# multimodallearning/convexAdam

Measured on AMD Instinct MI355X. Metric: volume-pairs/sec (160x192x224 MIND convex+Adam(80it)), higher is better.
Workload: dtype f32

## Files before the change

convexadam_amd/csrc/cvx_common.h:

```cpp
#pragma once
#include <hip/hip_runtime.h>
#include <stdint.h>
#include <stdio.h>
#include <stdarg.h>

#include <mutex>

#include "convexadam_hip.h"

namespace cvx {

void set_error(const char* fmt, ...);
int fail(int code, const char* fmt, ...);
int check_last(const char* what);

#define CVX_REQUIRE(cond, ...)                                      \
    do {                                                            \
        if (!(cond)) return ::cvx::fail(CVX_ERR_INVALID_ARG, __VA_ARGS__); \
    } while (0)

static inline hipStream_t as_stream(void* s) { return reinterpret_cast<hipStream_t>(s); }
static inline size_t align_up(size_t v, size_t a) { return (v + a - 1) / a * a; }
static inline int cdiv(int a, int b) { return (a + b - 1) / b; }
static inline int64_t cdiv64(int64_t a, int64_t b) { return (a + b - 1) / b; }

template <typename KernelT>
static inline void ensure_dynamic_lds(KernelT kernel, size_t bytes, size_t& granted) {
    static std::mutex mu;
    std::lock_guard<std::mutex> lock(mu);
    if (bytes > granted) {
        (void)hipFuncSetAttribute(reinterpret_cast<const void*>(kernel), hipFuncAttributeMaxDynamicSharedMemorySize, (int)bytes);
        (void)hipGetLastError();
        granted = bytes;
    }
}

struct Carver {
    char* base = nullptr;
    size_t used = 0;
    Carver() = default;
    explicit Carver(void* p) : base(static_cast<char*>(p)) {}
    size_t take_bytes(size_t bytes) { const size_t off = align_up(used, 256); used = off + bytes; return off; }
    template <typename T> T* take(size_t count) { const size_t off = take_bytes(count * sizeof(T)); return base ? reinterpret_cast<T*>(base + off) : nullptr; }
};
static inline size_t ws_query(const Carver& m) { return m.used ? m.used + 256 : 0; }

#define CVX_OPTIONS(X) \
    X(mind_tiled,          "CVX_MIND_TILED",            0)   \
    X(mind_overlap,        "CVX_MIND_OVERLAP",          0)   \
    X(mm_tx,               "CVX_MM_TX",                 0)   \
    X(mm_slots,            "CVX_MM_SLOTS",            512)   \
    X(box_tiled,           "CVX_BOX_TILED",             0)   \
    X(no_prune,            "CVX_NO_PRUNE",              0)   \
    X(corr_unfused,        "CVX_CORR_UNFUSED",          0)   \
    X(corr_fused_all,      "CVX_CORR_FUSED_ALL",        0)   \
    X(prune_stream_above,  "CVX_PRUNE_STREAM_ABOVE",   -1)   \
    X(cf_census,           "CVX_CF_CENSUS",             0)   \
    X(cf_prio,             "CVX_CF_PRIO",             136)   \
    X(warp_flat,           "CVX_WARP_FLAT",             0)   \
    X(box_yt,              "CVX_BOX_YT",                8)   \
    X(box_wg_target,       "CVX_BOX_WG_TARGET",         0)   \
    X(box_xsplit,          "CVX_BOX_XSPLIT",           -1)   \
    X(box_cpt,             "CVX_BOX_CPT",               4)   \
    X(box_uneven,          "CVX_BOX_UNEVEN",          200)   \
    X(box_adam_role,       "CVX_BOX_ADAM_ROLE",         0)   \
    X(box_dpp,             "CVX_BOX_DPP",               0)   \
    X(box_pk,              "CVX_BOX_PK",                0)   \
    X(box_prio,            "CVX_BOX_PRIO",              0)   \
    X(label_pow_block,     "CVX_LABEL_POW_BLOCK",      32)   \
    X(census_ptr,          nullptr,                     0)   \
    X(mind_mean_threads,   "CVX_MIND_MEAN_THREADS",     0)   \
    X(edt_sequential,      "CVX_EDT_SEQUENTIAL",        0)   \
    X(warp_octant,         "CVX_WARP_OCTANT",           4)   \
    X(box_fwd_tile,        "CVX_BOX_FWD_TILE",         -1)   \
    X(box_bwd_tile,        "CVX_BOX_BWD_TILE",         -1)   \
    X(box_walk,            "CVX_BOX_WALK",              1)   \
    X(corr_dual,           "CVX_CORR_DUAL",             0)   \
    X(prune_refine,        "CVX_PRUNE_REFINE",          1)   \
    X(mind_records,        "CVX_MIND_RECORDS",          1)   \
    X(resize_up2,          "CVX_RESIZE_UP2",            1)   \
    X(mind_blocked,        "CVX_MIND_BLOCKED",          1)   \
    X(corr_cert,           "CVX_CORR_CERT",             1)   \
    X(cc_debug,            "CVX_CC_DEBUG",              0)   \
    X(ic_fused,            "CVX_IC_FUSED",              0)   \
    X(mind_single,         "CVX_MIND_SINGLE",           0)   \
    X(ms_zlen,             "CVX_MS_ZLEN",               0)   \
    X(cf_map,              "CVX_CF_MAP",                1)   \
    X(cert_unfused,        "CVX_CERT_UNFUSED",          0)   \
    X(fbox_tile,           "CVX_FBOX_TILE",             0)   \
    X(box_tile_sync,       "CVX_BOX_TILE_SYNC",         0)   \
    X(box_prediv,          "CVX_BOX_PREDIV",            1)   \
    X(tile_census_ptr,     nullptr,                     0)
#define X(name, env, dflt) long long name;
struct Options { CVX_OPTIONS(X) };
#undef X
Options& options();
const unsigned* adam_sqrt_table();
class ContextScope {
public:
    explicit ContextScope(const cvx_context* c);
    ~ContextScope();
    ContextScope(const ContextScope&) = delete;
    ContextScope& operator=(const ContextScope&) = delete;
private:
    void* prev_;
    bool active_;
};

#ifdef CVX_RACE_JITTER
__device__ __forceinline__ void cvx_jitter() {
    unsigned t = (unsigned)__builtin_amdgcn_s_memtime();
    t ^= (unsigned)__builtin_amdgcn_s_getreg((4 << 0) | (0 << 6) | (31 << 11)) * 2654435761u;
    t ^= t >> 13; t *= 0x9E3779B1u; t ^= t >> 15;
    const int n = (int)(t & 15);
    for (int i = 0; i < n; ++i) __builtin_amdgcn_s_sleep(1);
}
__device__ __forceinline__ void cvx_barrier() { cvx_jitter(); __syncthreads(); cvx_jitter(); }
#else
__device__ __forceinline__ void cvx_barrier() { __syncthreads(); }
#endif

__device__ __forceinline__ int clampi(int v, int lo, int hi) { return v < lo ? lo : (v > hi ? hi : v); }

__device__ __forceinline__ float fdiv(float a, float b) { return __fdiv_rn(a, b); }
__device__ __forceinline__ float fsqrt(float a) { return sqrtf(a); }

__device__ __forceinline__ float cvx_expf(float d) {
    const float R_LN2f = 1.442695040888963407359924681001892137426645954152985934135449406931f;
    const float L2Uf = 0.693145751953125f, L2Lf = 1.428606765330187045e-06f;
    const float qf = rintf(d * R_LN2f);
    const int q = (int)qf;
    float s = __builtin_fmaf(qf, -L2Uf, d);
    s = __builtin_fmaf(qf, -L2Lf, s);
    float u = 0.000198527617612853646278381f;
    u = __builtin_fmaf(u, s, 0.00139304355252534151077271f);
    u = __builtin_fmaf(u, s, 0.00833336077630519866943359f);
    u = __builtin_fmaf(u, s, 0.0416664853692054748535156f);
    u = __builtin_fmaf(u, s, 0.166666671633720397949219f);
    u = __builtin_fmaf(u, s, 0.5f);
    u = 1.0f + __builtin_fmaf(s * s, u, s);
    u = __builtin_ldexpf(u, q);
    if (d < -104.0f) u = 0.0f;
    if (d > 100.0f) u = __int_as_float(0x7f800000);
    return u;
}

struct ExpTable { const unsigned char* tbl; unsigned first, count; };
ExpTable mind_exp_table();

typedef float f32x4 __attribute__((ext_vector_type(4)));
typedef __attribute__((address_space(3))) f32x4 lds_f32x4;
__device__ __forceinline__ f32x4 lds_load4(const float* p) { return *(const volatile lds_f32x4*)p; }
__device__ __forceinline__ void lds_store4(float* p, f32x4 v) { *(volatile lds_f32x4*)p = v; }

typedef int i32x4 __attribute__((ext_vector_type(4)));
__device__ __forceinline__ float4 buffer_load16(__amdgpu_buffer_rsrc_t rsrc, unsigned lane_off, unsigned uni_off) {
    const i32x4 v = __builtin_bit_cast(i32x4, __builtin_amdgcn_raw_buffer_load_b128(rsrc, (int)lane_off, (int)uni_off, 0));
    return make_float4(__int_as_float(v.x), __int_as_float(v.y), __int_as_float(v.z), __int_as_float(v.w));
}

typedef float f32x2 __attribute__((ext_vector_type(2)));
typedef __attribute__((address_space(3))) f32x2 lds_f32x2;
__device__ __forceinline__ f32x2 lds_load2(const float* p) { return *(const volatile lds_f32x2*)p; }
__device__ __forceinline__ void lds_store2(float* p, f32x2 v) { *(volatile lds_f32x2*)p = v; }

template <int D>
__device__ __forceinline__ float div_exact(float x) {
    static_assert(D == 8 || D == 27 || D == 64 || D == 125 || D == 343, "divisor not verified");
    constexpr float r = 1.0f / (float)D;
    const float q = x * r;
    const float e = __builtin_fmaf(-(float)D, q, x);
    return __builtin_fmaf(e, r, q);
}
template <int D>
__device__ __forceinline__ float div_exact_inf(float x) { return __builtin_isinf(x) ? x : div_exact<D>(x); }

template <int N>
__device__ __forceinline__ float cascade_seq(const float (&v)[N]) {
    static_assert(N < 256, "two cascade levels");
    float a0 = 0.f, a1 = 0.f;
    int i = 0;
#pragma unroll
    for (; i + 16 <= N; i += 16) {
#pragma unroll
        for (int j = 0; j < 16; ++j) a0 += v[i + j];
        a1 += a0;
        a0 = 0.f;
    }
#pragma unroll
    for (; i < N; ++i) a0 += v[i];
    a0 += a1;
    return a0;
}
template <int N>
__device__ __forceinline__ float outer_sum_ilp(const float (&v)[N]) {
    static_assert(N / 4 < 16, "single cascade level inside the interleaved sums");
    float p[4] = {0.f, 0.f, 0.f, 0.f};
#pragma unroll
    for (int i = 0; i < N / 4; ++i)
#pragma unroll
        for (int k = 0; k < 4; ++k) p[k] += v[4 * i + k];
#pragma unroll
    for (int i = (N / 4) * 4; i < N; ++i) p[0] += v[i];
    p[0] += p[1];
    p[0] += p[2];
    p[0] += p[3];
    return p[0];
}

__device__ __forceinline__ unsigned long long pack_min_key(float v, unsigned idx) {
    unsigned b = __float_as_uint(v);
    b = (b & 0x80000000u) ? ~b : (b | 0x80000000u);
    if (v != v) b = 0u;
    return ((unsigned long long)b << 32) | idx;
}

struct Tri {
    float ix, iy, iz;
    int x0, y0, z0;
    float tnw, tne, tsw, tse, bnw, bne, bsw, bse;
};
__device__ __forceinline__ float unnormalize(float g, int S) { return ((g + 1.0f) * (float)S - 1.0f) * 0.5f; }
__device__ __forceinline__ void tri_setup(Tri& t, float gx, float gy, float gz, int h, int w, int d) {
    t.ix = unnormalize(gx, d);
    t.iy = unnormalize(gy, w);
    t.iz = unnormalize(gz, h);
    const float fx = floorf(t.ix), fy = floorf(t.iy), fz = floorf(t.iz);
    t.x0 = (int)fmaxf(fminf(fx, 1.0e9f), -1.0e9f);
    t.y0 = (int)fmaxf(fminf(fy, 1.0e9f), -1.0e9f);
    t.z0 = (int)fmaxf(fminf(fz, 1.0e9f), -1.0e9f);
    const float x1 = (float)(t.x0 + 1), y1 = (float)(t.y0 + 1), z1 = (float)(t.z0 + 1);
    const float x0f = (float)t.x0, y0f = (float)t.y0, z0f = (float)t.z0;
    t.tnw = (x1 - t.ix) * (y1 - t.iy) * (z1 - t.iz);
    t.tne = (t.ix - x0f) * (y1 - t.iy) * (z1 - t.iz);
    t.tsw = (x1 - t.ix) * (t.iy - y0f) * (z1 - t.iz);
    t.tse = (t.ix - x0f) * (t.iy - y0f) * (z1 - t.iz);
    t.bnw = (x1 - t.ix) * (y1 - t.iy) * (t.iz - z0f);
    t.bne = (t.ix - x0f) * (y1 - t.iy) * (t.iz - z0f);
    t.bsw = (x1 - t.ix) * (t.iy - y0f) * (t.iz - z0f);
    t.bse = (t.ix - x0f) * (t.iy - y0f) * (t.iz - z0f);
}
__device__ __forceinline__ bool inb3(int z, int y, int x, int h, int w, int d) {
    return z >= 0 && z < h && y >= 0 && y < w && x >= 0 && x < d;
}
__device__ __forceinline__ float tri_sample(const Tri& t, const float* __restrict__ vol, int h, int w, int d) {
    const int x0 = t.x0, y0 = t.y0, z0 = t.z0, x1 = x0 + 1, y1 = y0 + 1, z1 = z0 + 1;
    const bool zi0 = (unsigned)z0 < (unsigned)h, zi1 = (unsigned)z1 < (unsigned)h, yi0 = (unsigned)y0 < (unsigned)w,
               yi1 = (unsigned)y1 < (unsigned)w, xi0 = (unsigned)x0 < (unsigned)d, xi1 = (unsigned)x1 < (unsigned)d;
    const int zc0 = clampi(z0, 0, h - 1), zc1 = clampi(z1, 0, h - 1), yc0 = clampi(y0, 0, w - 1), yc1 = clampi(y1, 0, w - 1),
              xc0 = clampi(x0, 0, d - 1), xc1 = clampi(x1, 0, d - 1);
    const size_t r00 = ((size_t)zc0 * w + yc0) * d, r01 = ((size_t)zc0 * w + yc1) * d, r10 = ((size_t)zc1 * w + yc0) * d,
                 r11 = ((size_t)zc1 * w + yc1) * d;
    const float v0 = vol[r00 + xc0], v1 = vol[r00 + xc1], v2 = vol[r01 + xc0], v3 = vol[r01 + xc1], v4 = vol[r10 + xc0],
                v5 = vol[r10 + xc1], v6 = vol[r11 + xc0], v7 = vol[r11 + xc1];
    float o = 0.0f, n;
    n = o + v0 * t.tnw; o = (zi0 && yi0 && xi0) ? n : o;
    n = o + v1 * t.tne; o = (zi0 && yi0 && xi1) ? n : o;
    n = o + v2 * t.tsw; o = (zi0 && yi1 && xi0) ? n : o;
    n = o + v3 * t.tse; o = (zi0 && yi1 && xi1) ? n : o;
    n = o + v4 * t.bnw; o = (zi1 && yi0 && xi0) ? n : o;
    n = o + v5 * t.bne; o = (zi1 && yi0 && xi1) ? n : o;
    n = o + v6 * t.bsw; o = (zi1 && yi1 && xi0) ? n : o;
    n = o + v7 * t.bse; o = (zi1 && yi1 && xi1) ? n : o;
    return o;
}

__device__ __forceinline__ void lin_coef(int o, int in, int out, int& i0, int& i1, float& l0, float& l1) {
    if (in == out) { i0 = o; i1 = o; l0 = 1.0f; l1 = 0.0f; return; }
    const float ratio = fdiv((float)in, (float)out);
    float src = __builtin_fmaf(ratio, (float)o + 0.5f, -0.5f);
    src = src < 0.0f ? 0.0f : src;
    int a = (int)floorf(src);
    a = a > in - 1 ? in - 1 : a;
    float l = src - (float)a;
    l = l < 0.f ? 0.f : (l > 1.f ? 1.f : l);
    i0 = a;
    i1 = a + ((a < in - 1) ? 1 : 0);
    l1 = l;
    l0 = 1.0f - l;
}
__device__ __forceinline__ float resize_chain(const float (&v)[8], float pre_mul, float lx0, float lx1, float ly0, float ly1, float lz0,
                                              float lz1) {
    const float a0 = __builtin_fmaf(v[0] * pre_mul, lx0, (v[1] * pre_mul) * lx1);
    const float a1 = __builtin_fmaf(v[2] * pre_mul, lx0, (v[3] * pre_mul) * lx1);
    const float b0 = __builtin_fmaf(v[4] * pre_mul, lx0, (v[5] * pre_mul) * lx1);
    const float b1 = __builtin_fmaf(v[6] * pre_mul, lx0, (v[7] * pre_mul) * lx1);
    const float l0 = __builtin_fmaf(a0, ly0, a1 * ly1);
    const float l1 = __builtin_fmaf(b0, ly0, b1 * ly1);
    return __builtin_fmaf(l0, lz0, l1 * lz1);
}

struct FastDiv { unsigned d, m; };
static inline FastDiv fastdiv_make(int d) { FastDiv f; f.d = (unsigned)d; f.m = d <= 1 ? 0u : (unsigned)((((unsigned long long)1 << 32) + (unsigned)d - 1) / (unsigned)d); return f; }
__device__ __forceinline__ int fastdiv(int n, FastDiv f) { return f.d <= 1 ? n : (int)__umulhi((unsigned)n, f.m); }

void profile_mark_kernel(const char* name, hipStream_t s);

int launch_box_zero(const float* in, float* out, int C, int H, int W, int D, int k, bool backward, hipStream_t s);
int launch_smoother(const float* in, float* out, float* tmp, int C, int H, int W, int D, const cvx_smoother& sm, bool backward,
                    hipStream_t s);
int launch_argmin_keys(const void* ssd, bool f16, int K, size_t v, unsigned long long* keys, bool arm, hipStream_t s);
struct CoupledWs { unsigned long long* keys[3]; int* idx; float* smin; unsigned long long* list; int* counts; };
CoupledWs coupled_layout(Carver& cv, int h, int w, int d, int disp_hw);
int launch_argmin(const void* ssd, bool f16, const float* mesh, const float* u, float coef, bool coupled, int K, size_t v,
                  unsigned long long* keys, int64_t* argmin_out, hipStream_t s);
int launch_resize(const float* in, int C, int h, int w, int d, float* out, int H, int W, int D, float pre_mul,
                  float post_div, hipStream_t s);
int launch_resize2(const float* in, int C, int h, int w, int d, int H, int W, int D, float* scratch, float* out, int h2, int w2,
                   int d2, float post_div, hipStream_t s);
struct AdamConsts { float w1, b2, omb2, bc2s, neg_step; const unsigned* sqrt_tbl; };
__device__ __forceinline__ float adam_sqrt(float x, const unsigned* __restrict__ tbl) {
    float r = fsqrt(x);
    if (tbl) {
        const unsigned b = __float_as_uint(x), e = b >> 23, mant = b & 0x7fffffu;
        if (b != 0 && e < 255) {
            const unsigned key = e ? (((e & 1u) << 23) | mant) : ((1u << 24) | mant);
            const unsigned code = (tbl[key >> 4] >> ((key & 15u) * 2u)) & 3u;
            if (code) r = __uint_as_float(__float_as_uint(r) + (code == 1u ? 1u : 0xffffffffu));
        }
    }
    return r;
}
__device__ __forceinline__ bool argmin_better(float cost, float best) { return (cost < best) | ((cost != cost) & (best == best)); }
__device__ __forceinline__ void adam_update(float g, float& P, float& m, float& v, const AdamConsts& ac) {
    const float mm = __builtin_fmaf(ac.w1, g - m, m);
    float vv = v * ac.b2;
    vv = __builtin_fmaf(ac.omb2 * g, g, vv);
    const float den = fdiv(adam_sqrt(vv, ac.sqrt_tbl), ac.bc2s) + 1e-8f;
    P = P + fdiv(ac.neg_step * mm, den);
    m = mm;
    v = vv;
}
struct AdamRun {
    const float *F2, *M2; int C, h, w, d; float *P, *m, *v; float lambda_weight; int niter, step0; float cost_scale;
    const float *base_h, *base_w, *base_d; float *U, *grad_out; const int* snapshot_iters_host; int n_snap; float* snapshots;
    void* workspace; size_t workspace_bytes; void* stream;
    const cvx_smoother* sm = nullptr;
    bool keep_state = true;
    bool f16_features = false;
    int fast = 0;
    bool features_are_records = false;
};
int adam_run_impl(const AdamRun& r);
size_t adam_record_floats(int C, size_t V);
int coupled_convex_impl(const void* ssd, bool f16, const int64_t* argmin, const float* mesh, int h, int w, int d, int disp_hw, float* out,
                        bool argmin_is_exact, void* workspace, size_t workspace_bytes, void* stream,
                        const unsigned char* cmask = nullptr);
int coupled_convex_dual_impl(const void* ssdA, const int64_t* argminA, float* outA, void* wsA, const void* ssdB, bool f16, const int64_t* argminB,
                             float* outB, void* wsB, const float* mesh, int h, int w, int d, int disp_hw, size_t workspace_bytes,
                             void* stream, bool counts_zeroed = false);
bool mind_pooled_supported(int H, int W, int D, int g1, int g2);
int launch_mind_pooled(const float* img, int H, int W, int D, int radius, int dilation, int g1, float* out1, int g2, float* out2,
                       float* raw, void* workspace, size_t workspace_bytes, hipStream_t s, int records = 0);
bool mind_pooled_records_supported(int H, int W, int D, int g1, int g2);
size_t mind_pooled_raw_floats(int H, int W, int D, int g1, int g2);
int launch_label_pooled(const float* lab, int H, int W, int D, int C, const int* present, const float* weights, float mult, int g1, float* out1,
                        int g2, float* out2, hipStream_t s);
bool corr_box2_supported(int h, int w, int d, int px);
int launch_corr_box2(const float* raw, int K, int h, int w, int d, int px, float* ssd, hipStream_t s, bool fast = false);
bool corr_fused_supported(int C, int h, int w, int d, int hw);
void corr_fused_set_prep_hook(void (*hook)(hipStream_t));
int corr_fused_items(int C, int h, int w, int d, int hw);
bool corr_fused_tiled(int C, int h, int w, int d, int hw);
void corr_call_prep_hook(hipStream_t s);
size_t corr_fused_workspace_bytes(int C, int h, int w, int d, int hw);
int launch_corr_fused(const float* fix, const float* mov, int C, int h, int w, int d, int hw, int cost, int n_box, int fast, int f16,
                      void* ssd, void* workspace, size_t workspace_bytes, hipStream_t s);
int launch_corr_fused_dual(const float* fix, const float* mov, int C, int h, int w, int d, int hw, int cost, int n_box, int fast, int f16,
                           void* ssd, void* ssd_rev, void* workspace, size_t workspace_bytes, void* workspace_rev, hipStream_t s);
bool corr_cert_supported(int C, int h, int w, int d, int hw);
size_t corr_cert_workspace_bytes(int C, int h, int w, int d, int hw);
int launch_corr_cert(const float* fix, const float* mov, int C, int h, int w, int d, int hw, float* ssdu, void* workspace, size_t workspace_bytes,
                     hipStream_t s);
enum class CorrKernel { None, Fused, Round1, CertRole, CertStaged, CertRound1 };
struct CorrUse { bool variant, ic, no_prune; };
struct CorrPlan {
    CorrKernel exact;
    CorrKernel cert;
    bool cert_supported;
    bool fused_ws, staged_ws, cert_round1_ws;
    bool pair_cert;
    bool pair_dual, pair_dual_ws;
};
CorrPlan corr_plan(int C, int h, int w, int d, int hw, CorrUse use = CorrUse{false, false, false});
size_t corr_certfast_workspace_bytes(int C, int h, int w, int d, int hw);
int launch_corr_certfast(const float* fix, const float* mov, int C, int h, int w, int d, int hw, float* ssdu, void* workspace, size_t workspace_bytes,
                         hipStream_t s);
size_t corr_certify_workspace_bytes(int C, int h, int w, int d, int hw, bool plain = false);
int corr_certified_argmin(const float* ssdu, const float* fix, const float* mov, int C, int h, int w, int d, int hw, int64_t* argmin,
                          void* workspace, size_t workspace_bytes, hipStream_t s);
int coupled_convex_cert_impl(const float* ssduA, const float* fixA, const float* movA, float* outA, void* wsA, const float* ssduB, const float* fixB,
                             const float* movB, float* outB, void* wsB, const float* mesh, int C, int h, int w, int d, int hw, size_t workspace_bytes,
                             hipStream_t s, int stage = 0);
bool box3_march_supported(int d);
int launch_box3_march(const float* in, float* out, int h, int w, int d, bool backward, float* P, float* m, float* v,
                      AdamConsts ac, float* gsave, hipStream_t s);
bool box3_tile_fwd_supported(const float* in, const float* out, int h, int w, int d);
int launch_box3_tile_fwd(const float* in, float* out, int h, int w, int d, int variant, hipStream_t s);
int box3_tile_fwd_auto(int h, int w, int d);
bool box3_tile_supported(const float* in, const float* out, int h, int w, int d, const float* P, const float* m, const float* v, const float* gsave);
int launch_box3_tile(const float* in, float* out, int h, int w, int d, int variant, bool backward, float* P, float* m, float* v, AdamConsts ac,
                     float* gsave, bool prediv, hipStream_t s);
int launch_to_chunked(const float* in, int C, size_t V, float* out, bool half, hipStream_t s);
int launch_warp_grad(const float* Fcl, const float* Mcl, int C, int h, int w, int d, const float* U, const float* bh,
                     const float* bw, const float* bd, float gsc, float cH, float cW, float cD, float* gU, bool half, bool prediv, hipStream_t s);
int launch_warp_grad_fast(const float* Fcl, const float* Mcl, int C, int h, int w, int d, const float* U, const float* bh,
                          const float* bw, const float* bd, float gsc, float cH, float cW, float cD, float* gU, bool half, hipStream_t s);
int launch_box3_fast(const float* in, float* out, int h, int w, int d, float* P, float* m, float* v, double bc1, double bc2,
                     float* gsave, hipStream_t s);
bool boxchain_fast_supported(const cvx_smoother& sm, int h, int w, int d);
int launch_boxchain_fast(const float* in, float* out, int h, int w, int d, const cvx_smoother& sm, bool reverse, hipStream_t s);
int launch_adam_update_fast(const float* G, float* P, float* m, float* v, size_t n, double bc1, double bc2, hipStream_t s);

}
```

convexadam_amd/csrc/warp.hip:

```cpp
#include "cvx_common.h"

namespace cvx {

__global__ __launch_bounds__(256) void k_to_chunked(const float* __restrict__ in, int C, size_t V, float* __restrict__ out) {
    const size_t p = (size_t)blockIdx.x * blockDim.x + threadIdx.x;
    if (p > V) return;
    const int c0 = 4 * (int)blockIdx.y;
    float4 r = make_float4(0.f, 0.f, 0.f, 0.f);
    if (p < V) {
        const float* src = in + (size_t)c0 * V + p;
        r.x = src[0];
        if (c0 + 1 < C) r.y = src[V];
        if (c0 + 2 < C) r.z = src[2 * V];
        if (c0 + 3 < C) r.w = src[3 * V];
    }
    reinterpret_cast<float4*>(out)[(size_t)blockIdx.y * (V + 1) + p] = r;
}

typedef _Float16 h16x4 __attribute__((ext_vector_type(4)));
__global__ __launch_bounds__(256) void k_to_chunked_h(const float* __restrict__ in, int C, size_t V, uint2* __restrict__ out) {
    const size_t p = (size_t)blockIdx.x * blockDim.x + threadIdx.x;
    if (p > V) return;
    const int c0 = 4 * (int)blockIdx.y;
    float4 r = make_float4(0.f, 0.f, 0.f, 0.f);
    if (p < V) {
        const float* src = in + (size_t)c0 * V + p;
        r.x = src[0];
        if (c0 + 1 < C) r.y = src[V];
        if (c0 + 2 < C) r.z = src[2 * V];
        if (c0 + 3 < C) r.w = src[3 * V];
    }
    const h16x4 o = {(_Float16)r.x, (_Float16)r.y, (_Float16)r.z, (_Float16)r.w};
    out[(size_t)blockIdx.y * (V + 1) + p] = __builtin_bit_cast(uint2, o);
}
__device__ __forceinline__ float4 buffer_load8h(__amdgpu_buffer_rsrc_t rsrc, unsigned lane_off, unsigned uni_off) {
    const h16x4 v = __builtin_bit_cast(h16x4, __builtin_amdgcn_raw_buffer_load_b64(rsrc, (int)lane_off, (int)uni_off, 0));
    return make_float4((float)v.x, (float)v.y, (float)v.z, (float)v.w);
}

template <bool BUF, bool HALF = false, bool PREDIV = false>
__global__ __launch_bounds__(256) void k_warp_grad(const float* __restrict__ F2, const float* __restrict__ M2, int C, int CP,
                                                   int h, int w, int d, const float* __restrict__ U,
                                                   const float* __restrict__ bh, const float* __restrict__ bw,
                                                   const float* __restrict__ bd, float gsc, float cH, float cW, float cD,
                                                   float* __restrict__ gU, unsigned long long* __restrict__ census, FastDiv dx, FastDiv dy,
                                                   float sc0, float sc1, float sc2) {
    const size_t V = (size_t)h * w * d;
    if (census && threadIdx.x == 0) {
        census[4 * blockIdx.x] = __builtin_amdgcn_s_memrealtime();
        census[4 * blockIdx.x + 3] = __builtin_amdgcn_s_getreg((4 << 0) | (0 << 6) | (31 << 11)) | ((unsigned long long)__builtin_amdgcn_s_getreg((20 << 0) | (0 << 6) | (31 << 11)) << 32);
    }
    const int ntx = (d + 15) / 16, nty = (w + 3) / 4, ntz = (h + 3) / 4;
    const int per_xcd = (int)(gridDim.x >> 3);
    const int bid = __builtin_amdgcn_readfirstlane((int)blockIdx.x);
    const int tile = (bid & 7) * per_xcd + (bid >> 3);
    if (tile >= ntx * nty * ntz) return;
    const int trow = fastdiv(tile, dx), tbz = fastdiv(trow, dy);
    const int tbx = tile - trow * ntx, tby = trow - tbz * nty;
    const int x = tbx * 16 + (threadIdx.x & 15), y = tby * 4 + ((threadIdx.x >> 4) & 3), z = tbz * 4 + (threadIdx.x >> 6);
    if (x >= d || y >= w || z >= h) return;
    const unsigned p = (unsigned)((z * w + y) * d + x);
    const float uH = U[p], uW = U[V + p], uD = U[2 * V + p];
    Tri t;
    tri_setup(t, bd[x] + fdiv(uD, sc2), bw[y] + fdiv(uW, sc1), bh[z] + fdiv(uH, sc0), h, w, d);
    const int x0 = t.x0, y0 = t.y0, z0 = t.z0, x1 = x0 + 1, y1 = y0 + 1, z1 = z0 + 1;
    const float fx0 = (float)x0, fy0 = (float)y0, fz0 = (float)z0, fx1 = (float)x1, fy1 = (float)y1, fz1 = (float)z1;
    const bool zin0 = (unsigned)z0 < (unsigned)h, zin1 = (unsigned)z1 < (unsigned)h, yin0 = (unsigned)y0 < (unsigned)w,
               yin1 = (unsigned)y1 < (unsigned)w, xin0 = (unsigned)x0 < (unsigned)d, xin1 = (unsigned)x1 < (unsigned)d;
    const int r00 = (z0 * w + y0) * d, r01 = (z0 * w + y1) * d, r10 = (z1 * w + y0) * d, r11 = (z1 * w + y1) * d;
    constexpr unsigned REC = HALF ? 8u : 16u;
    const unsigned zero_rec = (unsigned)V * REC;
    unsigned off[8];
    off[0] = (zin0 && yin0 && xin0) ? (unsigned)(r00 + x0) * REC : zero_rec; off[1] = (zin0 && yin0 && xin1) ? (unsigned)(r00 + x1) * REC : zero_rec;
    off[2] = (zin0 && yin1 && xin0) ? (unsigned)(r01 + x0) * REC : zero_rec; off[3] = (zin0 && yin1 && xin1) ? (unsigned)(r01 + x1) * REC : zero_rec;
    off[4] = (zin1 && yin0 && xin0) ? (unsigned)(r10 + x0) * REC : zero_rec; off[5] = (zin1 && yin0 && xin1) ? (unsigned)(r10 + x1) * REC : zero_rec;
    off[6] = (zin1 && yin1 && xin0) ? (unsigned)(r11 + x0) * REC : zero_rec; off[7] = (zin1 && yin1 && xin1) ? (unsigned)(r11 + x1) * REC : zero_rec;
    const float wgt[8] = {t.tnw, t.tne, t.tsw, t.tse, t.bnw, t.bne, t.bsw, t.bse};
    const float ax[8] = {fy1 - t.iy, fy1 - t.iy, t.iy - fy0, t.iy - fy0, fy1 - t.iy, fy1 - t.iy, t.iy - fy0, t.iy - fy0};
    const float bx[8] = {fz1 - t.iz, fz1 - t.iz, fz1 - t.iz, fz1 - t.iz, t.iz - fz0, t.iz - fz0, t.iz - fz0, t.iz - fz0};
    const float ay[8] = {fx1 - t.ix, t.ix - fx0, fx1 - t.ix, t.ix - fx0, fx1 - t.ix, t.ix - fx0, fx1 - t.ix, t.ix - fx0};
    const float bz[8] = {fy1 - t.iy, fy1 - t.iy, t.iy - fy0, t.iy - fy0, fy1 - t.iy, fy1 - t.iy, t.iy - fy0, t.iy - fy0};
    float gix = 0.f, giy = 0.f, giz = 0.f;
    const unsigned foff = p * REC;
    const unsigned chunk_bytes = (unsigned)(V + 1) * REC;
    const __amdgpu_buffer_rsrc_t mr = __builtin_amdgcn_make_buffer_rsrc(const_cast<float*>(M2), 0, (int)(chunk_bytes * (unsigned)(CP / 4)), 0x00020000);
    const __amdgpu_buffer_rsrc_t fr = __builtin_amdgcn_make_buffer_rsrc(const_cast<float*>(F2), 0, (int)(chunk_bytes * (unsigned)(CP / 4)), 0x00020000);
    unsigned coff = 0;
    for (int c0 = 0; c0 < CP / 4; ++c0, coff += chunk_bytes) {
        float vv[8][4], fv[4];
#pragma unroll
        for (int k = 0; k < 8; ++k) {
            const float4 q = HALF ? buffer_load8h(mr, off[k], coff) : BUF ? buffer_load16(mr, off[k], coff) : *reinterpret_cast<const float4*>(reinterpret_cast<const char*>(M2) + (size_t)c0 * chunk_bytes + off[k]);
            vv[k][0] = q.x; vv[k][1] = q.y; vv[k][2] = q.z; vv[k][3] = q.w;
        }
        const float4 fq = HALF ? buffer_load8h(fr, foff, coff) : BUF ? buffer_load16(fr, foff, coff) : *reinterpret_cast<const float4*>(reinterpret_cast<const char*>(F2) + (size_t)c0 * chunk_bytes + foff);
        fv[0] = fq.x; fv[1] = fq.y; fv[2] = fq.z; fv[3] = fq.w;
#pragma unroll
        for (int j = 0; j < 4; ++j) {
            float wv = 0.0f;
#pragma unroll
            for (int k = 0; k < 8; ++k) wv += vv[k][j] * wgt[k];
            const float df = wv - fv[j];
            const float gOut = gsc * (2.0f * df);
            gix -= vv[0][j] * ax[0] * bx[0] * gOut; giy -= vv[0][j] * ay[0] * bx[0] * gOut; giz -= vv[0][j] * ay[0] * bz[0] * gOut;
            gix += vv[1][j] * ax[1] * bx[1] * gOut; giy -= vv[1][j] * ay[1] * bx[1] * gOut; giz -= vv[1][j] * ay[1] * bz[1] * gOut;
            gix -= vv[2][j] * ax[2] * bx[2] * gOut; giy += vv[2][j] * ay[2] * bx[2] * gOut; giz -= vv[2][j] * ay[2] * bz[2] * gOut;
            gix += vv[3][j] * ax[3] * bx[3] * gOut; giy += vv[3][j] * ay[3] * bx[3] * gOut; giz -= vv[3][j] * ay[3] * bz[3] * gOut;
            gix -= vv[4][j] * ax[4] * bx[4] * gOut; giy -= vv[4][j] * ay[4] * bx[4] * gOut; giz += vv[4][j] * ay[4] * bz[4] * gOut;
            gix += vv[5][j] * ax[5] * bx[5] * gOut; giy -= vv[5][j] * ay[5] * bx[5] * gOut; giz += vv[5][j] * ay[5] * bz[5] * gOut;
            gix -= vv[6][j] * ax[6] * bx[6] * gOut; giy += vv[6][j] * ay[6] * bx[6] * gOut; giz += vv[6][j] * ay[6] * bz[6] * gOut;
            gix += vv[7][j] * ax[7] * bx[7] * gOut; giy += vv[7][j] * ay[7] * bx[7] * gOut; giz += vv[7][j] * ay[7] * bz[7] * gOut;
        }
    }
    float g[3];
    g[0] = fdiv(((float)h / 2.0f) * giz, sc0);
    g[1] = fdiv(((float)w / 2.0f) * giy, sc1);
    g[2] = fdiv(((float)d / 2.0f) * gix, sc2);
    const unsigned sH = (unsigned)(w * d);
    const unsigned pxp = x < d - 1 ? p + 1 : p, pxm = x > 0 ? p - 1 : p, pzp = z < h - 1 ? p + sH : p, pzm = z > 0 ? p - sH : p,
                   pyp = y < w - 1 ? p + (unsigned)d : p, pym = y > 0 ? p - (unsigned)d : p;
    float nb[3][6];
    const __amdgpu_buffer_rsrc_t ur = __builtin_amdgcn_make_buffer_rsrc(const_cast<float*>(U), 0, (int)(12u * (unsigned)V), 0x00020000);
    const unsigned nboff[6] = {4u * pxp, 4u * pxm, 4u * pzp, 4u * pzm, 4u * pyp, 4u * pym};
#pragma unroll
    for (int a = 0; a < 3; ++a)
#pragma unroll
        for (int k = 0; k < 6; ++k) nb[a][k] = __builtin_bit_cast(float, __builtin_amdgcn_raw_buffer_load_b32(ur, (int)nboff[k], (int)(4u * (unsigned)V) * a, 0));
    const float uc3[3] = {uH, uW, uD};
#pragma unroll
    for (int a = 0; a < 3; ++a) {
        const float uc = uc3[a];
        float acc = g[a], t;
        t = acc + -(cD * (2.0f * (nb[a][0] - uc))); acc = x < d - 1 ? t : acc;
        t = acc +  (cD * (2.0f * (uc - nb[a][1]))); acc = x > 0 ? t : acc;
        t = acc + -(cH * (2.0f * (nb[a][2] - uc))); acc = z < h - 1 ? t : acc;
        t = acc +  (cH * (2.0f * (uc - nb[a][3]))); acc = z > 0 ? t : acc;
        t = acc + -(cW * (2.0f * (nb[a][4] - uc))); acc = y < w - 1 ? t : acc;
        t = acc +  (cW * (2.0f * (uc - nb[a][5]))); acc = y > 0 ? t : acc;
        (gU + (size_t)a * V)[p] = PREDIV ? (acc == 0.0f ? acc : div_exact<27>(acc)) : acc;
    }
    if (census && threadIdx.x == 0) census[4 * blockIdx.x + 2] = __builtin_amdgcn_s_memrealtime();
}


int launch_to_chunked(const float* in, int C, size_t V, float* out, bool half, hipStream_t s) {
    const int CP = (C + 3) / 4 * 4;
    if ((size_t)(CP / 4) * (V + 1) * 16 >= ((size_t)1 << 31)) return fail(CVX_ERR_UNSUPPORTED, "adam_run: control grid too large (%zu voxels x %d channels)", V, C);
    if (half) hipLaunchKernelGGL(k_to_chunked_h, dim3((unsigned)cdiv64((int64_t)(V + 1), 256), CP / 4), dim3(256), 0, s, in, C, V, reinterpret_cast<uint2*>(out));
    else hipLaunchKernelGGL(k_to_chunked, dim3((unsigned)cdiv64((int64_t)(V + 1), 256), CP / 4), dim3(256), 0, s, in, C, V, out);
    return check_last("to_chunked");
}

int launch_warp_grad(const float* Fcl, const float* Mcl, int C, int h, int w, int d, const float* U, const float* bh,
                     const float* bw, const float* bd, float gsc, float cH, float cW, float cD, float* gU, bool half, bool prediv, hipStream_t s) {
    const int CP = (C + 3) / 4 * 4;
    const dim3 gv((unsigned)((cdiv(d, 16) * cdiv(w, 4) * cdiv(h, 4) + 7) / 8 * 8));
    unsigned long long* census = reinterpret_cast<unsigned long long*>(options().census_ptr);
    if (census) census += 8 * 1024;
    const FastDiv dx = fastdiv_make(cdiv(d, 16)), dy = fastdiv_make(cdiv(w, 4));
    const float sc0 = (float)((h - 1) / 2.0), sc1 = (float)((w - 1) / 2.0), sc2 = (float)((d - 1) / 2.0);
#define CVX_WG_LAUNCH(...) hipLaunchKernelGGL((k_warp_grad<__VA_ARGS__>), gv, dim3(256), 0, s, Fcl, Mcl, C, CP, h, w, d, U, bh, bw, bd, gsc, cH, cW, cD, gU, census, dx, dy, sc0, sc1, sc2)
    if (half) { if (prediv) CVX_WG_LAUNCH(true, true, true); else CVX_WG_LAUNCH(true, true); }
    else if (options().warp_flat) { if (prediv) CVX_WG_LAUNCH(false, false, true); else CVX_WG_LAUNCH(false); }
    else if (prediv) CVX_WG_LAUNCH(true, false, true);
    else CVX_WG_LAUNCH(true);
#undef CVX_WG_LAUNCH
    return check_last("warp_grad");
}

}
```

Measured before the change: 148.5.

## Double-buffer half-record loads in warp gradient and prefetch neighbour displacements early

In the buffer-load fp32 path of the warp-gradient kernel, each 16-byte channel record is split into two 8-byte halves. Loads are software-pipelined so one half's gathers are in flight while the other half is accumulated. The 18 neighbour displacement loads for the regulariser are issued before the final accumulation so their latency overlaps compute. This aims to hide gather latency but doubles the number of load instructions and raises register pressure from two live record buffers.

Result: slower. 145.6 (-2.0%).

```diff
diff --git a/convexadam_amd/csrc/cvx_common.h b/convexadam_amd/csrc/cvx_common.h
--- a/convexadam_amd/csrc/cvx_common.h
+++ b/convexadam_amd/csrc/cvx_common.h
@@ -157,6 +157,12 @@
 __device__ __forceinline__ float4 buffer_load16(__amdgpu_buffer_rsrc_t rsrc, unsigned lane_off, unsigned uni_off) {
     const i32x4 v = __builtin_bit_cast(i32x4, __builtin_amdgcn_raw_buffer_load_b128(rsrc, (int)lane_off, (int)uni_off, 0));
     return make_float4(__int_as_float(v.x), __int_as_float(v.y), __int_as_float(v.z), __int_as_float(v.w));
+}
+
+typedef int i32x2 __attribute__((ext_vector_type(2)));
+__device__ __forceinline__ float2 buffer_load8(__amdgpu_buffer_rsrc_t rsrc, unsigned lane_off, unsigned uni_off) {
+    const i32x2 v = __builtin_bit_cast(i32x2, __builtin_amdgcn_raw_buffer_load_b64(rsrc, (int)lane_off, (int)uni_off, 0));
+    return make_float2(__int_as_float(v.x), __int_as_float(v.y));
 }
 
 typedef float f32x2 __attribute__((ext_vector_type(2)));
diff --git a/convexadam_amd/csrc/warp.hip b/convexadam_amd/csrc/warp.hip
--- a/convexadam_amd/csrc/warp.hip
+++ b/convexadam_amd/csrc/warp.hip
@@ -85,47 +85,81 @@
     const unsigned chunk_bytes = (unsigned)(V + 1) * REC;
     const __amdgpu_buffer_rsrc_t mr = __builtin_amdgcn_make_buffer_rsrc(const_cast<float*>(M2), 0, (int)(chunk_bytes * (unsigned)(CP / 4)), 0x00020000);
     const __amdgpu_buffer_rsrc_t fr = __builtin_amdgcn_make_buffer_rsrc(const_cast<float*>(F2), 0, (int)(chunk_bytes * (unsigned)(CP / 4)), 0x00020000);
-    unsigned coff = 0;
-    for (int c0 = 0; c0 < CP / 4; ++c0, coff += chunk_bytes) {
-        float vv[8][4], fv[4];
-#pragma unroll
-        for (int k = 0; k < 8; ++k) {
-            const float4 q = HALF ? buffer_load8h(mr, off[k], coff) : BUF ? buffer_load16(mr, off[k], coff) : *reinterpret_cast<const float4*>(reinterpret_cast<const char*>(M2) + (size_t)c0 * chunk_bytes + off[k]);
-            vv[k][0] = q.x; vv[k][1] = q.y; vv[k][2] = q.z; vv[k][3] = q.w;
-        }
-        const float4 fq = HALF ? buffer_load8h(fr, foff, coff) : BUF ? buffer_load16(fr, foff, coff) : *reinterpret_cast<const float4*>(reinterpret_cast<const char*>(F2) + (size_t)c0 * chunk_bytes + foff);
-        fv[0] = fq.x; fv[1] = fq.y; fv[2] = fq.z; fv[3] = fq.w;
-#pragma unroll
-        for (int j = 0; j < 4; ++j) {
-            float wv = 0.0f;
-#pragma unroll
-            for (int k = 0; k < 8; ++k) wv += vv[k][j] * wgt[k];
-            const float df = wv - fv[j];
-            const float gOut = gsc * (2.0f * df);
-            gix -= vv[0][j] * ax[0] * bx[0] * gOut; giy -= vv[0][j] * ay[0] * bx[0] * gOut; giz -= vv[0][j] * ay[0] * bz[0] * gOut;
-            gix += vv[1][j] * ax[1] * bx[1] * gOut; giy -= vv[1][j] * ay[1] * bx[1] * gOut; giz -= vv[1][j] * ay[1] * bz[1] * gOut;
-            gix -= vv[2][j] * ax[2] * bx[2] * gOut; giy += vv[2][j] * ay[2] * bx[2] * gOut; giz -= vv[2][j] * ay[2] * bz[2] * gOut;
-            gix += vv[3][j] * ax[3] * bx[3] * gOut; giy += vv[3][j] * ay[3] * bx[3] * gOut; giz -= vv[3][j] * ay[3] * bz[3] * gOut;
-            gix -= vv[4][j] * ax[4] * bx[4] * gOut; giy -= vv[4][j] * ay[4] * bx[4] * gOut; giz += vv[4][j] * ay[4] * bz[4] * gOut;
-            gix += vv[5][j] * ax[5] * bx[5] * gOut; giy -= vv[5][j] * ay[5] * bx[5] * gOut; giz += vv[5][j] * ay[5] * bz[5] * gOut;
-            gix -= vv[6][j] * ax[6] * bx[6] * gOut; giy += vv[6][j] * ay[6] * bx[6] * gOut; giz += vv[6][j] * ay[6] * bz[6] * gOut;
-            gix += vv[7][j] * ax[7] * bx[7] * gOut; giy += vv[7][j] * ay[7] * bx[7] * gOut; giz += vv[7][j] * ay[7] * bz[7] * gOut;
-        }
-    }
-    float g[3];
-    g[0] = fdiv(((float)h / 2.0f) * giz, sc0);
-    g[1] = fdiv(((float)w / 2.0f) * giy, sc1);
-    g[2] = fdiv(((float)d / 2.0f) * gix, sc2);
+    auto channel = [&](const auto& vv, const int j, const float fj) {
+        float wv = 0.0f;
+#pragma unroll
+        for (int k = 0; k < 8; ++k) wv += vv[k][j] * wgt[k];
+        const float df = wv - fj;
+        const float gOut = gsc * (2.0f * df);
+        gix -= vv[0][j] * ax[0] * bx[0] * gOut; giy -= vv[0][j] * ay[0] * bx[0] * gOut; giz -= vv[0][j] * ay[0] * bz[0] * gOut;
+        gix += vv[1][j] * ax[1] * bx[1] * gOut; giy -= vv[1][j] * ay[1] * bx[1] * gOut; giz -= vv[1][j] * ay[1] * bz[1] * gOut;
+        gix -= vv[2][j] * ax[2] * bx[2] * gOut; giy += vv[2][j] * ay[2] * bx[2] * gOut; giz -= vv[2][j] * ay[2] * bz[2] * gOut;
+        gix += vv[3][j] * ax[3] * bx[3] * gOut; giy += vv[3][j] * ay[3] * bx[3] * gOut; giz -= vv[3][j] * ay[3] * bz[3] * gOut;
+        gix -= vv[4][j] * ax[4] * bx[4] * gOut; giy -= vv[4][j] * ay[4] * bx[4] * gOut; giz += vv[4][j] * ay[4] * bz[4] * gOut;
+        gix += vv[5][j] * ax[5] * bx[5] * gOut; giy -= vv[5][j] * ay[5] * bx[5] * gOut; giz += vv[5][j] * ay[5] * bz[5] * gOut;
+        gix -= vv[6][j] * ax[6] * bx[6] * gOut; giy += vv[6][j] * ay[6] * bx[6] * gOut; giz += vv[6][j] * ay[6] * bz[6] * gOut;
+        gix += vv[7][j] * ax[7] * bx[7] * gOut; giy += vv[7][j] * ay[7] * bx[7] * gOut; giz += vv[7][j] * ay[7] * bz[7] * gOut;
+    };
     const unsigned sH = (unsigned)(w * d);
     const unsigned pxp = x < d - 1 ? p + 1 : p, pxm = x > 0 ? p - 1 : p, pzp = z < h - 1 ? p + sH : p, pzm = z > 0 ? p - sH : p,
                    pyp = y < w - 1 ? p + (unsigned)d : p, pym = y > 0 ? p - (unsigned)d : p;
     float nb[3][6];
     const __amdgpu_buffer_rsrc_t ur = __builtin_amdgcn_make_buffer_rsrc(const_cast<float*>(U), 0, (int)(12u * (unsigned)V), 0x00020000);
     const unsigned nboff[6] = {4u * pxp, 4u * pxm, 4u * pzp, 4u * pzm, 4u * pyp, 4u * pym};
-#pragma unroll
-    for (int a = 0; a < 3; ++a)
-#pragma unroll
-        for (int k = 0; k < 6; ++k) nb[a][k] = __builtin_bit_cast(float, __builtin_amdgcn_raw_buffer_load_b32(ur, (int)nboff[k], (int)(4u * (unsigned)V) * a, 0));
+    auto request_nb = [&]() {
+#pragma unroll
+        for (int a = 0; a < 3; ++a)
+#pragma unroll
+            for (int k = 0; k < 6; ++k) nb[a][k] = __builtin_bit_cast(float, __builtin_amdgcn_raw_buffer_load_b32(ur, (int)nboff[k], (int)(4u * (unsigned)V) * a, 0));
+    };
+    if constexpr (BUF && !HALF) {
+        struct HalfRec { float v[8][2], f[2]; };
+        auto request = [&](HalfRec& r, const unsigned uni) {
+#pragma unroll
+            for (int k = 0; k < 8; ++k) {
+                const float2 q = buffer_load8(mr, off[k], uni);
+                r.v[k][0] = q.x; r.v[k][1] = q.y;
+            }
+            const float2 fq = buffer_load8(fr, foff, uni);
+            r.f[0] = fq.x; r.f[1] = fq.y;
+        };
+        auto sum = [&](const HalfRec& r) {
+#pragma unroll
+            for (int j = 0; j < 2; ++j) channel(r.v, j, r.f[j]);
+        };
+        HalfRec A, B;
+        unsigned coff = 0;
+        request(A, 0u);
+        for (int c0 = 1; c0 < CP / 4; ++c0, coff += chunk_bytes) {
+            request(B, coff + 8u);
+            sum(A);
+            request(A, coff + chunk_bytes);
+            sum(B);
+        }
+        request(B, coff + 8u);
+        sum(A);
+        request_nb();
+        sum(B);
+    } else {
+        unsigned coff = 0;
+        for (int c0 = 0; c0 < CP / 4; ++c0, coff += chunk_bytes) {
+            float vv[8][4], fv[4];
+#pragma unroll
+            for (int k = 0; k < 8; ++k) {
+                const float4 q = HALF ? buffer_load8h(mr, off[k], coff) : *reinterpret_cast<const float4*>(reinterpret_cast<const char*>(M2) + (size_t)c0 * chunk_bytes + off[k]);
+                vv[k][0] = q.x; vv[k][1] = q.y; vv[k][2] = q.z; vv[k][3] = q.w;
+            }
+            const float4 fq = HALF ? buffer_load8h(fr, foff, coff) : *reinterpret_cast<const float4*>(reinterpret_cast<const char*>(F2) + (size_t)c0 * chunk_bytes + foff);
+            fv[0] = fq.x; fv[1] = fq.y; fv[2] = fq.z; fv[3] = fq.w;
+#pragma unroll
+            for (int j = 0; j < 4; ++j) channel(vv, j, fv[j]);
+        }
+        request_nb();
+    }
+    float g[3];
+    g[0] = fdiv(((float)h / 2.0f) * giz, sc0);
+    g[1] = fdiv(((float)w / 2.0f) * giy, sc1);
+    g[2] = fdiv(((float)d / 2.0f) * gix, sc2);
     const float uc3[3] = {uH, uW, uD};
 #pragma unroll
     for (int a = 0; a < 3; ++a) {
```
